# rqhuang88/DV-Matcher

Measured on AMD Instinct MI355X. Metric: point-cloud pairs/sec (N=2048, d=128), higher is better.
Workload: dtype f32; 1 GPU; BASELINE configs[1]: synthetic random pairs N=M=2048 d=128, correspondence+deform forward, both directions; deformer_weights=reference ckpt/dvmatcher_scape_r (fixture), fps_start=0, parallelism=pairs sharded over 1 GPU(s), no collective

## Files before the change

dv-matcher_amd/csrc/dvm_api.cpp:

```cpp
#include <stdarg.h>

#include "dvm_common.h"

namespace dvm {
static thread_local char g_err[512] = "";
void set_error(const char *fmt, ...) {
    va_list ap;
    va_start(ap, fmt);
    vsnprintf(g_err, sizeof(g_err), fmt, ap);
    va_end(ap);
}
}

DVM_EXPORT int dvm_abi_version(void) { return DVM_ABI_VERSION; }
DVM_EXPORT const char *dvm_last_error(void) { return dvm::g_err; }
DVM_EXPORT int dvm_device_count(void) {
    int n = 0;
    if (hipGetDeviceCount(&n) != hipSuccess) return 0;
    return n;
}

#include <atomic>
#include <stdlib.h>
namespace dvm {
// ... 13 lines not shown
static std::atomic<int> g_deterministic{options().deterministic};
bool deterministic() { return g_deterministic.load(std::memory_order_relaxed) != 0; }
}
DVM_EXPORT int dvm_set_deterministic(int on) { return dvm::g_deterministic.exchange(on ? 1 : 0); }
DVM_EXPORT int dvm_get_deterministic(void) { return dvm::g_deterministic.load(std::memory_order_relaxed); }

#include <map>
#include <mutex>
#include <utility>
namespace dvm {
static std::mutex g_attr_mu;
static std::map<std::pair<int, const void *>, int> g_attr_bytes;
void ensure_dyn_lds(const void *kernel, int bytes) {
    int dev = 0;
    if (hipGetDevice(&dev) != hipSuccess) return;
    std::lock_guard<std::mutex> lock(g_attr_mu);
    auto it = g_attr_bytes.find({dev, kernel});
    if (it != g_attr_bytes.end() && it->second >= bytes) return;
    if (hipFuncSetAttribute(kernel, hipFuncAttributeMaxDynamicSharedMemorySize, bytes) == hipSuccess) g_attr_bytes[{dev, kernel}] = bytes;
}
int device_cu_count() {
    static std::mutex mu;
    static std::map<int, int> cus;
    int dev = 0;
    if (hipGetDevice(&dev) != hipSuccess) return 256;
    std::lock_guard<std::mutex> lock(mu);
    auto it = cus.find(dev);
    if (it != cus.end()) return it->second;
    int n = 0;
    if (hipDeviceGetAttribute(&n, hipDeviceAttributeMultiprocessorCount, dev) != hipSuccess || n < 1) n = 256;
    cus[dev] = n;
    return n;
}
}

namespace dvm {
static std::mutex g_pair_mu;
static std::map<std::pair<int, hipStream_t>, PairCtx *> g_pair_ctx;
PairCtx *pair_ctx_find(hipStream_t caller) {
    int dev = 0;
    if (hipGetDevice(&dev) != hipSuccess) return nullptr;
    std::lock_guard<std::mutex> lock(g_pair_mu);
    auto it = g_pair_ctx.find({dev, caller});
    return it == g_pair_ctx.end() ? nullptr : it->second;
}
static void pair_ctx_free(PairCtx *c) {
    if (c->side) (void)hipStreamDestroy(c->side);
    if (c->side2) (void)hipStreamDestroy(c->side2);
    for (hipEvent_t e : {c->ev_fork, c->ev_join, c->ev_join2, c->ev_aux})
        if (e) (void)hipEventDestroy(e);
    delete c;
}
}

DVM_EXPORT int dvm_pair_init(void *stream) {
    int dev = 0;
    if (hipGetDevice(&dev) != hipSuccess) {
        dvm::set_error("dvm_pair_init: no current device");
        return DVM_ELAUNCH;
    }
    std::lock_guard<std::mutex> lock(dvm::g_pair_mu);
    const auto key = std::make_pair(dev, (hipStream_t)stream);
    if (dvm::g_pair_ctx.count(key)) return DVM_OK;
    dvm::PairCtx *c = new dvm::PairCtx();
    c->device = dev;
    if (hipStreamCreateWithFlags(&c->side, hipStreamNonBlocking) != hipSuccess ||
        hipStreamCreateWithFlags(&c->side2, hipStreamNonBlocking) != hipSuccess ||
// ... 150 lines not shown
```

dv-matcher_amd/csrc/dvm_common.h:

```cpp
#pragma once
#include <hip/hip_runtime.h>
#include <stdint.h>
#include <stdio.h>
#include <string.h>

#include "../../include/dvm.h"

#define DVM_EXPORT extern "C" __attribute__((visibility("default")))

namespace dvm {

void set_error(const char *fmt, ...);
void prof_begin(hipStream_t s, int id = 0);
void prof_end(hipStream_t s, int id = 0);
bool deterministic();
void prof_note(int id, const char *name);
void ensure_dyn_lds(const void *kernel, int bytes);
int device_cu_count();
struct Options {
    int deterministic;
    int k1_route;
    float k1_p_coarse, k1_p_lean;
    int linear_cfg;
    int pair_overlap;
    int debug;
};
constexpr int DVM_DEBUG_K1_ROUTES = 1, DVM_DEBUG_K1_FLAGGED = 2, DVM_DEBUG_CHAMFER_STATS = 4, DVM_DEBUG_K1_STAMPS = 8, DVM_DEBUG_MLP_STAMPS = 16;
const Options &options();
struct PairCtx {
    int device = 0;
    hipStream_t side = nullptr, side2 = nullptr;
    hipEvent_t ev_fork = nullptr, ev_join = nullptr, ev_join2 = nullptr, ev_aux = nullptr;
};
PairCtx *pair_ctx_find(hipStream_t caller);

#define DVM_REQUIRE(cond, ...)            \
    do {                                  \
        if (!(cond)) {                    \
            dvm::set_error(__VA_ARGS__);  \
            return DVM_EINVAL;            \
        }                                 \
    } while (0)

#define DVM_CHECK_LAUNCH(name)                                                          \
    do {                                                                                \
        hipError_t e_ = hipGetLastError();                                              \
        if (e_ != hipSuccess) {                                                         \
            dvm::set_error("%s: launch failed: %s", name, hipGetErrorString(e_));       \
            return DVM_ELAUNCH;                                                         \
        }                                                                               \
    } while (0)
// ... 392 lines not shown
```

dv-matcher_amd/csrc/dvm_deformer.hip:

```cpp
#include "dvm_mfma_tile.h"
#include "dvm_mlp_f16.h"

namespace dvm {


constexpr int DF_C = 128;

__global__ __launch_bounds__(256) void pool_kernel(const float *__restrict__ feat, const int32_t *__restrict__ idx,
                                                   const int32_t *__restrict__ rowmap, int P, int nrows, int k,
                                                   const float *__restrict__ cw, const float *__restrict__ cb,
                                                   float *__restrict__ out, int out_stride, int out_off,
                                                   const int32_t *__restrict__ order) {
    const int b = blockIdx.y;
    const long g = (long)blockIdx.x * blockDim.x + threadIdx.x;
    if (g >= (long)nrows * (DF_C / 4)) return;
    int r = (int)(g / (DF_C / 4));
    const int c4 = (int)(g % (DF_C / 4));
    if (order) r = order[(size_t)b * nrows + r];
    const int v = rowmap ? rowmap[(size_t)b * nrows + r] : r;
    const float *fb = feat + (size_t)b * P * DF_C;
    const int32_t *ix = idx + ((size_t)b * P + v) * k;
    f32x4 acc = {0.f, 0.f, 0.f, 0.f};
    if (k == 10) {
        int nb[10];
// ... 84 lines not shown
    } else {
#pragma unroll
        for (int t = 0; t < TOPK; ++t) {
            if (t < topk) {
                f32x4 f = *(const f32x4 *)(g2b + (size_t)pc[t] * DF_C + 4 * c4);
                acc.x = fmaf(pv[t], f.x, acc.x);
                acc.y = fmaf(pv[t], f.y, acc.y);
                acc.z = fmaf(pv[t], f.z, acc.z);
                acc.w = fmaf(pv[t], f.w, acc.w);
            }
        }
    }
    float *zr = z + ((size_t)b * Nn + n) * DF_ZS;
    zr[134 + 4 * c4] = acc.x, zr[135 + 4 * c4] = acc.y, zr[136 + 4 * c4] = acc.z, zr[137 + 4 * c4] = acc.w;
    if (c4 == 0) {
        for (int c = 0; c < 3; ++c) {
            zr[c] = verts1[row * 3 + c];
            zr[131 + c] = verts12[row * 3 + c];
        }
        zr[262] = 0.f, zr[263] = 0.f;
    }
}

struct AssembleSide {
    const float *vsrc, *vcorr, *gsrc, *gtgt, *pi_val;
    const int32_t *pi_idx, *fps;
    int N, M, Nn;
    float *z;
};
struct AssembleArgs {
    AssembleSide d[2];
    int topk;
    const int *gate;
};
template <int TOPK, bool PLANES = false>
__global__ __launch_bounds__(256) void assemble_pooled_kernel(const AssembleArgs args) {
    const int *__restrict__ gate = args.gate;
    if (gate && *gate == 0) return;
    const AssembleSide &A = args.d[blockIdx.z];
    const float *__restrict__ vsrc = A.vsrc, *__restrict__ vcorr = A.vcorr, *__restrict__ gsrc = A.gsrc, *__restrict__ gtgt = A.gtgt;
    const float *__restrict__ pi_val = A.pi_val;
    const int32_t *__restrict__ pi_idx = A.pi_idx, *__restrict__ fps = A.fps;
    const int N = A.N, M = A.M, Nn = A.Nn, topk = args.topk;
    float *__restrict__ z = A.z;
    const int b = blockIdx.y;
    const long g = (long)blockIdx.x * blockDim.x + threadIdx.x;
    if (g >= (long)Nn * (DF_C / 4)) return;
    const int n = (int)(g / (DF_C / 4)), c4 = (int)(g % (DF_C / 4));
    const int v = fps[(size_t)b * Nn + n];
    const size_t row = (size_t)b * N + v;
    const int lane = threadIdx.x & 63, base = lane & 32, l32 = lane & 31;
    const bool live = l32 < topk;
    const size_t o = row * topk + (live ? l32 : 0);
    const float pvt = pi_val[o];
    const int pct = pi_idx[o];
    const float my_pv = live ? pvt : 0.f;
    const int my_pc = live ? pct : 0x7fffffff;
    int rank = 0;
#pragma unroll
    for (int u = 0; u < TOPK; ++u) {
        const int pcu = __shfl(my_pc, base + u, 64);
        rank += (pcu < my_pc || (pcu == my_pc && u < l32)) ? 1 : 0;
    }
    const int dst = l32 < TOPK ? base + rank : lane;
    const int spc = __builtin_amdgcn_ds_permute(dst << 2, my_pc);
    const float spv = __int_as_float(__builtin_amdgcn_ds_permute(dst << 2, __float_as_int(my_pv)));
    float pv[TOPK];
    int pc[TOPK];
#pragma unroll
    for (int t = 0; t < TOPK; ++t) {
        pc[t] = __shfl(spc, base + t, 64);
        pv[t] = __shfl(spv, base + t, 64);
    }
    const float *gt = gtgt + (size_t)b * M * DF_C;
    f32x4 acc = {0.f, 0.f, 0.f, 0.f};
    if (topk == TOPK) {
        f32x4 f[TOPK];
#pragma unroll
        for (int t = 0; t < TOPK; ++t) f[t] = *(const f32x4 *)(gt + (size_t)pc[t] * DF_C + 4 * c4);
// ... 21 lines not shown
        typedef unsigned u32x2 __attribute__((ext_vector_type(2)));
        typedef unsigned u32x4 __attribute__((ext_vector_type(4)));
        char *zr = (char *)z + ((size_t)b * Nn + n) * MH_SZ;
        unsigned h0, m0, h1, m1;
        split2x2(gs.x * MH_SA, gs.y * MH_SA, h0, m0);
        split2x2(gs.z * MH_SA, gs.w * MH_SA, h1, m1);
        *(u32x2 *)(zr + 8 * c4) = u32x2{h0, h1};
        *(u32x2 *)(zr + 2 * MH_K0 + 8 * c4) = u32x2{m0, m1};
        split2x2(acc.x * MH_SA, acc.y * MH_SA, h0, m0);
        split2x2(acc.z * MH_SA, acc.w * MH_SA, h1, m1);
        *(u32x2 *)(zr + 256 + 8 * c4) = u32x2{h0, h1};
        *(u32x2 *)(zr + 2 * MH_K0 + 256 + 8 * c4) = u32x2{m0, m1};
        if (c4 == 0) {
            unsigned h2, m2;
            split2x2(vsrc[row * 3] * MH_SA, vsrc[row * 3 + 1] * MH_SA, h0, m0);
            split2x2(vsrc[row * 3 + 2] * MH_SA, vcorr[row * 3] * MH_SA, h1, m1);
            split2x2(vcorr[row * 3 + 1] * MH_SA, vcorr[row * 3 + 2] * MH_SA, h2, m2);
            *(u32x4 *)(zr + 512) = u32x4{h0, h1, h2, 0u};
            *(u32x4 *)(zr + 528) = u32x4{0u, 0u, 0u, 0u};
            *(u32x4 *)(zr + 2 * MH_K0 + 512) = u32x4{m0, m1, m2, 0u};
            *(u32x4 *)(zr + 2 * MH_K0 + 528) = u32x4{0u, 0u, 0u, 0u};
        }
        return;
    }
    float *zr = z + ((size_t)b * Nn + n) * DF_ZS;
    zr[3 + 4 * c4] = gs.x, zr[4 + 4 * c4] = gs.y, zr[5 + 4 * c4] = gs.z, zr[6 + 4 * c4] = gs.w;
    zr[134 + 4 * c4] = acc.x, zr[135 + 4 * c4] = acc.y, zr[136 + 4 * c4] = acc.z, zr[137 + 4 * c4] = acc.w;
    if (c4 == 0) {
        for (int c = 0; c < 3; ++c) {
            zr[c] = vsrc[row * 3 + c];
            zr[131 + c] = vcorr[row * 3 + c];
        }
        zr[262] = 0.f, zr[263] = 0.f;
    }
}

__device__ __forceinline__ float elu1(float x) { return x > 0.f ? x : __builtin_amdgcn_exp2f(x * 1.4426950408889634f) - 1.f; }

__global__ void mlp_layer_scalar_kernel(const float *__restrict__ in, int in_stride, const float *__restrict__ W,
                                        const float *__restrict__ bias, int rows, int I, int O, int act,
                                        float *__restrict__ out, int out_stride) {
    long g = (long)blockIdx.x * blockDim.x + threadIdx.x;
    if (g >= (long)rows * O) return;
    int r = (int)(g / O), o = (int)(g % O);
    const float *x = in + (size_t)r * in_stride, *w = W + (size_t)o * I;
    float acc = 0.f;
    for (int c = 0; c < I; ++c) acc = fmaf(x[c], w[c], acc);
    acc = acc + bias[o];
    out[(size_t)r * out_stride + o] = act ? elu1(acc) : acc;
}

__global__ void pack_weights_kernel(const float *__restrict__ W, int O, int I, int otiles, int steps, float *__restrict__ Wp) {
    long g = (long)blockIdx.x * blockDim.x + threadIdx.x;
    long total = (long)otiles * steps * 64;
    if (g >= total) return;
    int lane = (int)(g % 64);
    int step = (int)((g / 64) % steps);
    int ot = (int)(g / (64L * steps));
    int o = ot * 32 + (lane & 31), c = 2 * step + (lane >> 5);
    Wp[g] = (o < O && c < I) ? W[(size_t)o * I + c] : 0.f;
}

constexpr int ML_NODES = 32;
constexpr int ML_WAVES = 8;
constexpr int ML_THREADS = 64 * ML_WAVES;
constexpr int ML_SA = 268;
// ... 149 lines not shown
        layer(w.h0, 512, W1, b1, 512, 256, 1, w.h1, 256);
        layer(w.h1, 256, W2, b2, 256, 128, 1, w.h2, 128);
        layer(w.h2, 128, W3, b3, 128, 9, 0, out, 9);
    } else {
        launch_mlp_rows(w.z, rows, W0, b0, W1, b1, W2, b2, W3, b3, w.Wp0, out, s, variant, w.zp);
    }
    return DVM_OK;
}

__global__ void pad_rows_kernel(const float *__restrict__ in, int rows, int I, int stride, float *__restrict__ out) {
    long g = (long)blockIdx.x * blockDim.x + threadIdx.x;
    if (g >= (long)rows * stride) return;
    int r = (int)(g / stride), c = (int)(g % stride);
    out[g] = c < I ? in[(size_t)r * I + c] : 0.f;
}

void launch_pool_all(const float *feat, const int32_t *idx, int B, int P, int k, const float *cw, const float *cb, float *out,
                     hipStream_t s, const int32_t *order) {
    prof_begin(s, DVM_PROF_POOL);
    hipLaunchKernelGGL(pool_kernel, dim3((unsigned)(((long)P * 32 + 255) / 256), B), dim3(256), 0, s, feat, idx,
                       (const int32_t *)nullptr, P, P, k, cw, cb, out, DF_C, 0, order);
    prof_end(s, DVM_PROF_POOL);
}
void launch_assemble_pooled_pair(const float *verts1, const float *verts2, const float *verts12, const float *verts21, const float *g1,
                                 const float *g2, const float *val12, const int32_t *idx12, const float *val21, const int32_t *idx21,
                                 const int32_t *nodes1, const int32_t *nodes2, int B, int N, int M, void *z12, void *z21, bool planes,
                                 const int *gate, hipStream_t s) {
    AssembleArgs a;
    a.d[0] = AssembleSide{verts1, verts12, g1, g2, val12, idx12, nodes1, N, M, N / 2, (float *)z12};
    a.d[1] = AssembleSide{verts2, verts21, g2, g1, val21, idx21, nodes2, M, N, M / 2, (float *)z21};
    a.topk = 10, a.gate = gate;
    const int nn = N / 2 > M / 2 ? N / 2 : M / 2;
    const dim3 grid((unsigned)(((long)nn * 32 + 255) / 256), B, 2);
    if (!gate) prof_begin(s, DVM_PROF_ASSEMBLE);
    if (planes) hipLaunchKernelGGL((assemble_pooled_kernel<10, true>), grid, dim3(256), 0, s, a);
    else hipLaunchKernelGGL(assemble_pooled_kernel<10>, grid, dim3(256), 0, s, a);
    if (!gate) prof_end(s, DVM_PROF_ASSEMBLE);
}
const int *launch_mlp_planes(const void *zp, int rows, const float *W0, const float *b0, const float *W1, const float *b1, const float *W2,
                             const float *b2, const float *W3, const float *b3, float *wp, float *out, hipStream_t s) {
    return launch_mlp_planes_f16(zp, rows, W0, b0, W1, b1, W2, b2, W3, b3, wp, out, s);
}
void launch_mlp_fallback(const float *z, int rows, const float *W0, const float *b0, const float *W1, const float *b1, const float *W2,
                         const float *b2, const float *W3, const float *b3, float *wp, float *out, hipStream_t s, const int *flag) {
    launch_mlp_rows_bf16(z, rows, W0, b0, W1, b1, W2, b2, W3, b3, (char *)wp + mlp_f16_pack_bytes(), out, s, flag);
}
size_t mlp_pack_floats() {
    size_t f32 = (size_t)16 * 132 * 64 + (size_t)8 * 256 * 64 + (size_t)4 * 128 * 64 + (size_t)64 * 64;
    size_t h16 = (mlp_f16_pack_bytes() + mlp_bf16_pack_bytes() + 3) / 4;
    return f32 > h16 ? f32 : h16;
}
void launch_mlp_rows(const float *z, int rows, const float *W0, const float *b0, const float *W1, const float *b1, const float *W2,
                     const float *b2, const float *W3, const float *b3, float *wp, float *out, hipStream_t s, int variant, void *zp) {
    if (variant == 0 && zp) {
        launch_split_rows(z, rows, DF_ZS, zp, s);
        const int *flag = launch_mlp_planes_f16(zp, rows, W0, b0, W1, b1, W2, b2, W3, b3, wp, out, s);
        launch_mlp_rows_bf16(z, rows, W0, b0, W1, b1, W2, b2, W3, b3, (char *)wp + mlp_f16_pack_bytes(), out, s, flag);
        return;
    }
    if (variant == 0) variant = 3;
    if (variant == 3) {
        launch_mlp_rows_bf16(z, rows, W0, b0, W1, b1, W2, b2, W3, b3, wp, out, s, nullptr);
        return;
    }
    float *Wp0 = wp, *Wp1 = Wp0 + (size_t)16 * 132 * 64, *Wp2 = Wp1 + (size_t)8 * 256 * 64, *Wp3 = Wp2 + (size_t)4 * 128 * 64;
    auto pack = [&](const float *W, int O, int I, int otiles, int steps, float *Wp) {
        long th = (long)otiles * steps * 64;
        hipLaunchKernelGGL(pack_weights_kernel, dim3((unsigned)((th + 255) / 256)), dim3(256), 0, s, W, O, I, otiles, steps, Wp);
    };
// ... 56 lines not shown
```

dv-matcher_amd/csrc/dvm_mlp_bf16.hip:

```cpp
#include "dvm_mfma_tile.h"

namespace dvm {

typedef __bf16 bf16x8 __attribute__((ext_vector_type(8)));

constexpr int MB_NODES = 32, MB_WAVES = 8, MB_THREADS = 64 * MB_WAVES;
constexpr int MB_ZS = 264;
constexpr int MB_K0 = 272, MB_K1 = 512, MB_K2 = 256, MB_K3 = 128;
constexpr int MB_SA = 3 * MB_K0 * 2 + 16;
constexpr int MB_SB = 3 * MB_K1 * 2 + 16;
constexpr size_t MB_LDS_BYTES = (size_t)MB_NODES * (MB_SA + MB_SB);

__device__ __forceinline__ void split3(float x, __bf16 &h, __bf16 &m, __bf16 &l) {
    h = (__bf16)x;
    float r = x - (float)h;
    m = (__bf16)r;
    float r2 = r - (float)m;
    l = (__bf16)r2;
}

struct PackLayersBf16 {
    const float *W[4];
    int O[4], I[4], otiles[4], steps[4];
    __bf16 *Wp[4];
// ... 41 lines not shown
        acc = __builtin_amdgcn_mfma_f32_32x32x16_bf16(ah, bm, acc, 0, 0, 0);
        acc = __builtin_amdgcn_mfma_f32_32x32x16_bf16(ah, bh, acc, 0, 0, 0);
        bh = ch, bm = cm, bl = cl;
        ch = nh, cm = nm, cl = nl;
    }
    return acc;
}

__device__ __forceinline__ float elu_fast(float x) {
    return x > 0.f ? x : __builtin_amdgcn_exp2f(x * 1.4426950408889634f) - 1.f;
}

__device__ __forceinline__ void mlp_store_bf16(const f32x16 &acc, const float *__restrict__ bias, int o, int O, char *dst,
                                               int stride, int plane_bytes, int hh) {
    if (o >= O) return;
    const float bv = bias[o];
#pragma unroll
    for (int r = 0; r < 16; ++r) {
        const int node = lane_key(r, hh);
        __bf16 h, m, l;
        split3(elu_fast(acc[r] + bv), h, m, l);
        char *p = dst + node * stride + 2 * o;
        *(__bf16 *)(p) = h;
        *(__bf16 *)(p + plane_bytes) = m;
        *(__bf16 *)(p + 2 * plane_bytes) = l;
    }
}

__global__ __launch_bounds__(MB_THREADS) void mlp_bf16x3_kernel(const float *__restrict__ z, int rows,
                                                                const __bf16 *__restrict__ Wp0, const float *__restrict__ b0,
                                                                const __bf16 *__restrict__ Wp1, const float *__restrict__ b1,
                                                                const __bf16 *__restrict__ Wp2, const float *__restrict__ b2,
                                                                const __bf16 *__restrict__ Wp3, const float *__restrict__ b3,
                                                                float *__restrict__ out, const int *__restrict__ gate) {
    if (gate && *gate == 0) return;
    extern __shared__ __attribute__((aligned(16))) char smem[];
    char *bufA = smem;
    char *bufB = smem + MB_NODES * MB_SA;
    const int tid = threadIdx.x, lane = tid & 63, wave = tid >> 6;
    const int r32 = lane & 31, hh = lane >> 5;
    const int row0 = blockIdx.x * MB_NODES;

    for (int e = tid; e < MB_NODES * (MB_K0 / 4); e += MB_THREADS) {
        const int r = e / (MB_K0 / 4), c = e % (MB_K0 / 4);
        f32x4 v = {0.f, 0.f, 0.f, 0.f};
        if (row0 + r < rows && 4 * c < MB_ZS) v = *(const f32x4 *)(z + (size_t)(row0 + r) * MB_ZS + 4 * c);
        char *p = bufA + r * MB_SA + 8 * c;
#pragma unroll
        for (int q = 0; q < 4; ++q) {
            __bf16 h, m, l;
            split3(v[q], h, m, l);
            *(__bf16 *)(p + 2 * q) = h;
            *(__bf16 *)(p + 2 * MB_K0 + 2 * q) = m;
            *(__bf16 *)(p + 4 * MB_K0 + 2 * q) = l;
        }
    }
    __syncthreads();
    for (int q = 0; q < 2; ++q) {
        const int ot = wave * 2 + q;
        f32x16 acc = mlp_tile_bf16(bufA + r32 * MB_SA + 16 * hh, 2 * MB_K0, Wp0 + (size_t)ot * (MB_K0 / 16) * 1536 + lane * 8,
                                   MB_K0 / 16);
        mlp_store_bf16(acc, b0, ot * 32 + r32, 512, bufB, MB_SB, 2 * MB_K1, hh);
    }
    __syncthreads();
    {
        const int ot = wave;
        f32x16 acc = mlp_tile_bf16(bufB + r32 * MB_SB + 16 * hh, 2 * MB_K1, Wp1 + (size_t)ot * (MB_K1 / 16) * 1536 + lane * 8,
                                   MB_K1 / 16);
        mlp_store_bf16(acc, b1, ot * 32 + r32, 256, bufA, MB_SA, 2 * MB_K2, hh);
    }
    __syncthreads();
    if (wave < 4) {
        const int ot = wave;
        f32x16 acc = mlp_tile_bf16(bufA + r32 * MB_SA + 16 * hh, 2 * MB_K2, Wp2 + (size_t)ot * (MB_K2 / 16) * 1536 + lane * 8,
                                   MB_K2 / 16);
        mlp_store_bf16(acc, b2, ot * 32 + r32, 128, bufB, MB_SB, 2 * MB_K3, hh);
    }
    __syncthreads();
    if (wave == 0) {
        f32x16 acc = mlp_tile_bf16(bufB + r32 * MB_SB + 16 * hh, 2 * MB_K3, Wp3 + lane * 8, MB_K3 / 16);
        const int o = r32;
        const float bv = o < 9 ? b3[o] : 0.f;
#pragma unroll
        for (int r = 0; r < 16; ++r) {
            const int node = lane_key(r, hh);
            if (o < 9 && row0 + node < rows) out[(size_t)(row0 + node) * 9 + o] = acc[r] + bv;
        }
    }
}

size_t mlp_bf16_pack_bytes() {
    return align_up(((size_t)16 * (MB_K0 / 16) + (size_t)8 * (MB_K1 / 16) + (size_t)4 * (MB_K2 / 16) + (size_t)1 * (MB_K3 / 16)) * 1536 *
                    sizeof(__bf16));
}

void launch_mlp_rows_bf16(const float *z, int rows, const float *W0, const float *b0, const float *W1, const float *b1,
                          const float *W2, const float *b2, const float *W3, const float *b3, void *scratch, float *out,
                          hipStream_t s, const int *gate) {
    __bf16 *Wp0 = (__bf16 *)scratch;
    __bf16 *Wp1 = Wp0 + (size_t)16 * (MB_K0 / 16) * 1536;
    __bf16 *Wp2 = Wp1 + (size_t)8 * (MB_K1 / 16) * 1536;
    __bf16 *Wp3 = Wp2 + (size_t)4 * (MB_K2 / 16) * 1536;
    {
        PackLayersBf16 a;
        long maxth = 0;
        auto layer = [&](int q, const float *W, int O, int I, int otiles, int steps, __bf16 *Wp) {
            a.W[q] = W, a.O[q] = O, a.I[q] = I, a.otiles[q] = otiles, a.steps[q] = steps, a.Wp[q] = Wp;
            const long th = (long)otiles * steps * 512;
            maxth = th > maxth ? th : maxth;
        };
        layer(0, W0, 512, 262, 16, MB_K0 / 16, Wp0);
        layer(1, W1, 256, 512, 8, MB_K1 / 16, Wp1);
        layer(2, W2, 128, 256, 4, MB_K2 / 16, Wp2);
        layer(3, W3, 9, 128, 1, MB_K3 / 16, Wp3);
        hipLaunchKernelGGL(pack_layers_bf16_kernel, dim3((unsigned)((maxth + 255) / 256), 4), dim3(256), 0, s, a, gate);
    }
    ensure_dyn_lds((const void *)mlp_bf16x3_kernel, (int)MB_LDS_BYTES);
    hipLaunchKernelGGL(mlp_bf16x3_kernel, dim3((rows + MB_NODES - 1) / MB_NODES), dim3(MB_THREADS), MB_LDS_BYTES, s, z, rows, Wp0,
                       b0, Wp1, b1, Wp2, b2, Wp3, b3, out, gate);
}

}
```

dv-matcher_amd/csrc/dvm_softcorr_coarse.hip:

```cpp
#include <stdlib.h>

#include "dvm_softcorr_f16.h"

namespace dvm {
namespace k1 {
namespace {

constexpr int HC_ROWB = 256;
constexpr int HC_KL = 12;
constexpr unsigned HC_REMOVED = 0xffc00000u;
constexpr unsigned HC_KBASE = 129u << 23;
constexpr float HC_FLOOR = 4.5f;
constexpr unsigned HC_EMASK = 0xffffe00fu;
constexpr int HC_MAX_M = 256 * 32;

constexpr int HC_QB = 2;
constexpr int HC_NREC = 32;
constexpr int HC_WAVES = 4;
template <int KT, int W> constexpr int hc_lds_bytes() { return 2 * KT * HC_ROWB + 2 * KT * 32 + 1024 + W * HC_QB * HC_NREC * 64 * 2; }

struct HCGroup {
    const char *qp, *kp;
    const char *knf;
    const float *nq;
// ... 126 lines not shown
#pragma unroll
        for (int s = 0; s < 8; ++s) qh[qb][s] = -*(const f16x8 *)(qptr + 32 * s);
        const float nas = norm_scaled(G.nq[(size_t)b * N + qrc], se);
        const float nasb = (nas + nas * 0x1p-8f) + HC_FLOOR;
        rowc[qb] = nasb - nas;
        qn[qb] = f16x8{0, 0, 0, 0, 0, 0, 0, 0};
        if (h == 0) {
            _Float16 p1, p2, p3;
            norm_pieces(nasb, p1, p2, p3);
            qn[qb][0] = (_Float16)0x1p+15f, qn[qb][1] = (_Float16)0x1p+4f, qn[qb][2] = (_Float16)0x1p-7f;
            qn[qb][3] = p1, qn[qb][4] = p2, qn[qb][5] = p3;
        }
    }

    List32<HC_KL> kb[QB];
#pragma unroll
    for (int qb = 0; qb < QB; ++qb) kb[qb].init();

    const int ntiles = (M + KT - 1) / KT, nsub = SUBS * ntiles;
    const int rgrp = (nsub + NREC - 1) / NREC;
    unsigned short *const rec = rec0 + (size_t)wave * QB * NREC * 64 + lane;
    unsigned urec[QB];
#pragma unroll
    for (int qb = 0; qb < QB; ++qb) urec[qb] = 0xffffffffu;

    const __amdgpu_buffer_rsrc_t krs = __builtin_amdgcn_make_buffer_rsrc((void *)kbase, 0, M * HB_ROWB, 0x00020000);
    const __amdgpu_buffer_rsrc_t nrs = __builtin_amdgcn_make_buffer_rsrc((void *)nfbase, 0, G.Mpad * 32, 0x00020000);
    auto stage_tile = [&](int t, int buf, bool clamp) __attribute__((always_inline)) {
        int lane;
        asm volatile("v_mbcnt_lo_u32_b32 %0, -1, 0\n\tv_mbcnt_hi_u32_b32 %0, -1, %0" : "=v"(lane));
        const int j0 = t * KT;
        char *kt = ktile0 + (size_t)buf * KT * HC_ROWB;
        constexpr int PIECES = KT * HC_ROWB / 1024 / W, NP = KT * 32 / 1024;
#pragma unroll
        for (int e = 0; e < PIECES; ++e) {
            const int piece = wave * PIECES + e;
            const int r = 4 * piece + (lane >> 4), rc = clamp ? min(r, M - 1 - j0) : r;
            const unsigned off = rc * HB_ROWB + (((lane & 15) ^ (r & 15)) << 4);
            __builtin_amdgcn_raw_ptr_buffer_load_lds(krs, (__attribute__((address_space(3))) void *)(kt + piece * 1024), 16, off, j0 * HB_ROWB, 0, 0);
        }
        __builtin_amdgcn_raw_ptr_buffer_load_lds(nrs, (__attribute__((address_space(3))) void *)(wave < NP ? knf0 + buf * KT * 32 + wave * 1024 : dump0), 16,
                                                 (wave < NP ? wave : 0) * 1024 + lane * 16, j0 * 32, 0, 0);
    };
    auto dma_barrier = [&]() __attribute__((always_inline)) {
        asm volatile("s_waitcnt vmcnt(0)" ::: "memory");
        __syncthreads();
    };

    unsigned fadr[8];
    {
        const unsigned rowb = (unsigned)(size_t)(const __attribute__((address_space(3))) char *)ktile0 + r32 * HC_ROWB;
        const int tq = h ^ (r32 & 15);
#pragma unroll
        for (int s = 0; s < 8; ++s) {
            fadr[s] = rowb + (((2 * s) ^ tq) << 4);
            asm volatile("" : "+v"(fadr[s]));
        }
    }
    unsigned nadr = (unsigned)(size_t)(const __attribute__((address_space(3))) char *)knf0 + r32 * 32 + 16 * h;
    asm volatile("" : "+v"(nadr));
    auto lds16 = [](unsigned adr, int off) __attribute__((always_inline)) {
        return *(const f16x8 *)(const __attribute__((address_space(3))) char *)(size_t)(adr + off);
    };
    struct Acc {
        f32x16 a[QB];
    };
    auto chain = [&](int buf, int sub) __attribute__((always_inline)) -> Acc {
        const int toff = buf * (KT * HC_ROWB) + sub * (32 * HC_ROWB);
        Acc A;
#pragma unroll
        for (int qb = 0; qb < QB; ++qb) A.a[qb] = f32x16{0.f, 0.f, 0.f, 0.f, 0.f, 0.f, 0.f, 0.f, 0.f, 0.f, 0.f, 0.f, 0.f, 0.f, 0.f, 0.f};
#pragma unroll
        for (int s = 0; s < 8; ++s) {
            const f16x8 fr = lds16(fadr[s], toff);
#pragma unroll
// ... 335 lines not shown
```

dv-matcher_amd/csrc/dvm_softcorr_f16.hip:

```cpp
#include "dvm_softcorr_f16.h"

namespace dvm {
namespace {

using namespace k1;

template <bool LEAN, bool CHECK_ROUTE = true>
__device__ __forceinline__ void sweep_f16_block(const HBArgs &args, int block, int nblocks, char *smem_b) {
    char *const ktile0 = smem_b;
    float *const knorm0 = (float *)(smem_b + (size_t)2 * HB_KT * HB_ROWB);
    float *const stage = knorm0 + 2 * HB_KT + (threadIdx.x >> 6) * HB_STAGE + (threadIdx.x & 63);

    int lid = xcd_remap(block, nblocks);
    const int grp = lid >= args.blocks0 ? 1 : 0;
    lid -= grp ? args.blocks0 : 0;
    const HBGroup &G = args.g[grp];
    const int N = G.N, M = G.M;
    const int b = lid / G.tiles, qt = lid % G.tiles;
    if (CHECK_ROUTE && args.route && args.route[grp * args.nb + b] != (LEAN ? K1_ROUTE_LEAN : K1_ROUTE_FULL)) return;
    const float neg_alpha = args.neg_alpha;
    const int tid = threadIdx.x, lane = tid & 63, wave = tid >> 6;
    const int r32 = lane & 31, h = lane >> 5;

    const char *kbase = G.kp + (size_t)b * M * HB_ROWB;
// ... 149 lines not shown
        __syncthreads();
    }

    {
        const float co = __shfl_xor(cref, 32, 64), lo = __shfl_xor(l, 32, 64);
        const float cm = fmaxf(cref, co);
        const float a = (cref == -INFINITY) ? 0.f : l * exp2f((cref - cm) * LOG2E);
        const float bb = (co == -INFINITY) ? 0.f : lo * exp2f((co - cm) * LOG2E);
        l = a + bb;
        cref = cm;
        double other[HB_KC];
#pragma unroll
        for (int t = 0; t < HB_KC; ++t)
            other[t] = __hiloint2double(__shfl_xor(__double2hiint(kb.e[t]), 32, 64), __shfl_xor(__double2loint(kb.e[t]), 32, 64));
#pragma unroll
        for (int t = 0; t < HB_KC; ++t) add_term(PackedBest<HB_KC>::key_of(kb.insert(other[t])));
    }
    if (h == 0 && qrow < N) {
        const size_t row = (size_t)b * N + qrow;
#pragma unroll
        for (int t = 0; t < HB_KC; ++t) {
            G.cidx[row * HB_KC + t] = PackedBest<HB_KC>::col_of(kb.e[t]);
            G.cd2[row * HB_KC + t] = kb.key(t);
        }
        G.lsum[row * 2] = l;
        G.lsum[row * 2 + 1] = cref;
    }
}
template <bool LEAN>
__global__ __launch_bounds__(HB_THREADS, 2) void softcorr_sweep_f16_kernel(const HBArgs args) {
    extern __shared__ __attribute__((aligned(16))) char smem_b[];
    sweep_f16_block<LEAN>(args, blockIdx.x, gridDim.x, smem_b);
}
__global__ __launch_bounds__(HB_THREADS, 2) void softcorr_sweep_f16_routed_kernel(const HBArgs args) {
    extern __shared__ __attribute__((aligned(16))) char smem_b[];
    int lid = xcd_remap(blockIdx.x, gridDim.x);
    const int grp = lid >= args.blocks0 ? 1 : 0;
    lid -= grp ? args.blocks0 : 0;
    const int route = args.route[grp * args.nb + lid / args.g[grp].tiles];
    if (route == K1_ROUTE_LEAN) sweep_f16_block<true, false>(args, blockIdx.x, gridDim.x, smem_b);
    else if (route == K1_ROUTE_FULL) sweep_f16_block<false, false>(args, blockIdx.x, gridDim.x, smem_b);
}
__global__ __launch_bounds__(HB_THREADS, 2) void softcorr_sweep_f16_gated_kernel(const HBArgs args, int nblocks) {
    extern __shared__ __attribute__((aligned(16))) char smem_b[];
    const bool on0 = args.route[0] == K1_ROUTE_LEAN, on1 = nblocks > args.blocks0 && args.route[args.nb] == K1_ROUTE_LEAN;
    if (!on0 && !on1) return;
    for (int vb = blockIdx.x; vb < nblocks; vb += gridDim.x) {
        sweep_f16_block<true>(args, vb, nblocks, smem_b);
        __syncthreads();
    }
}

}

void k1::launch_sweep_f16(const HBArgs &a, int blocks, int form, hipStream_t s) {
    auto go = [&](auto kernel, int grid, auto... more) {
        ensure_dyn_lds((const void *)kernel, (int)HB_LDS_BYTES);
        hipLaunchKernelGGL(kernel, dim3(grid), dim3(HB_THREADS), HB_LDS_BYTES, s, a, more...);
    };
    if (form == K1_SWEEP_ROUTED) go(softcorr_sweep_f16_routed_kernel, blocks);
    else if (form == K1_SWEEP_GATED) go(softcorr_sweep_f16_gated_kernel, blocks < 2048 ? blocks : 2048, blocks);
    else if (form == K1_ROUTE_LEAN) go(softcorr_sweep_f16_kernel<true>, blocks);
    else go(softcorr_sweep_f16_kernel<false>, blocks);
}

}
```

include/dvm.h:

```cpp
#ifndef DVM_H
#define DVM_H

#include <stddef.h>
#include <stdint.h>

#ifdef __cplusplus
extern "C" {
#endif

#define DVM_ABI_VERSION 1

#define DVM_OK 0
#define DVM_EINVAL (-1)
#define DVM_ELAUNCH (-2)
#define DVM_ENOSPACE (-3)

typedef int (*dvm_allreduce_fn)(void *user, void *buf, size_t count, int dtype, int op, void *stream);
typedef struct dvm_collective {
    dvm_allreduce_fn allreduce;
    void *user;
} dvm_collective;


int dvm_abi_version(void);
// ... 8 lines not shown
#define DVM_PROF_KNN_XYZ 5
#define DVM_PROF_FPS 6
#define DVM_PROF_ASSEMBLE 7
#define DVM_PROF_COUNT 8
int dvm_profile_enable(int max_launches);
int dvm_profile_select(unsigned kernel_mask);
int dvm_profile_read(double *total_ms, int *launches);
int dvm_profile_read_kernel(int kernel, double *total_ms, int *launches);
const char *dvm_profile_kernel_name(int kernel);
int dvm_profile_disable(void);

int dvm_rownorm2_f32(const float *x, int rows, int K, float *out, void *stream);

int dvm_linear_f32(const float *x, const float *w, int B, int N, int K, int Co, int channel_major, const float *bias,
                   const float *res, const float *bn_alpha, const float *bn_beta, float slope, float *y, void *stream);

int dvm_linear_prefix_f32(const float *xg, int Cg, const float *x, const float *w, int B, int N, int K, int Co,
                          const float *bias, const float *res, const float *bn_alpha, const float *bn_beta, float slope,
                          float *y, void *stream);

int dvm_linear_scaled_residual_f32(const float *x, const float *w, int B, int N, int K, int Co, int channel_major, const float *bias,
                                   float scale, const float *res, float *y, void *stream);

int dvm_linear_last_launch(int *info);

int dvm_linear_wgrad_f32(const float *gy, const float *x, long R, int Co, int K, float *dW, void *stream);
size_t dvm_linear_wgrad_workspace_bytes(long R, int Co, int K);
int dvm_linear_wgrad_ws_f32(const float *gy, const float *x, long R, int Co, int K, float *dW, void *ws, size_t ws_bytes, void *stream);

int dvm_set_deterministic(int on);
int dvm_get_deterministic(void);

int dvm_k1_last_routes(int *counts);

size_t dvm_softcorr_workspace_bytes(int B, int N, int M, int d);
int dvm_softcorr_fwd_f32(const float *f1, const float *f2, int B, int N, int M, int d, float neg_alpha, int topk,
                         float *pi_val, int32_t *pi_idx, float *row_smax, float *row_sum, int variant, void *ws,
                         size_t ws_bytes, void *stream);

size_t dvm_sinkhorn_workspace_bytes(int B, int N, int M, int d);
int dvm_sinkhorn_fwd_f32(const float *f1, const float *f2, int B, int N, int M, int d, float neg_alpha, int n_iter,
                         int topk, float *pi_val, int32_t *pi_idx, float *row_lmax, float *row_sum, float *u, float *v,
                         int variant, void *ws, size_t ws_bytes, void *stream);

size_t dvm_sinkhorn_hist_workspace_bytes(int B, int N, int M, int d);
int dvm_sinkhorn_fwd_hist_f32(const float *f1, const float *f2, int B, int N, int M, int d, float neg_alpha, int n_iter,
                              int topk, float *pi_val, int32_t *pi_idx, float *row_lmax, float *row_sum, float *u_hist,
                              float *v_hist, int variant, void *ws, size_t ws_bytes, void *stream);
size_t dvm_sinkhorn_bwd_workspace_bytes(int B, int N, int M, int d, int n_iter);
int dvm_sinkhorn_bwd_f32(const float *f1, const float *f2, int B, int N, int M, int d, float neg_alpha, int n_iter, int topk,
                         const float *pi_val, const int32_t *pi_idx, const float *u_hist, const float *v_hist,
                         const float *g_val, float *d_f1, float *d_f2, int variant, void *ws, size_t ws_bytes,
                         void *stream);

size_t dvm_sinkhorn_ub_workspace_bytes(int B, int N, int M, int d);
int dvm_sinkhorn_ub_fwd_f32(const float *f1, const float *f2, int B, int N, int M, int d, float neg_alpha, int n_iter, int topk,
                            float tau_row, float tau_col, const float *log_a, const float *log_b, float *pi_val,
                            int32_t *pi_idx, float *row_lmax, float *row_sum, float *row_lmass, float *u, float *v, int variant,
                            void *ws, size_t ws_bytes, void *stream);
size_t dvm_sinkhorn_ub_hist_workspace_bytes(int B, int N, int M, int d);
int dvm_sinkhorn_ub_fwd_hist_f32(const float *f1, const float *f2, int B, int N, int M, int d, float neg_alpha, int n_iter,
                                 int topk, float tau_row, float tau_col, const float *log_a, const float *log_b, float *pi_val,
                                 int32_t *pi_idx, float *row_lmax, float *row_sum, float *row_lmass, float *rn_hist,
                                 float *cn_hist, int variant, void *ws, size_t ws_bytes, void *stream);
size_t dvm_sinkhorn_ub_bwd_workspace_bytes(int B, int N, int M, int d, int n_iter);
int dvm_sinkhorn_ub_bwd_f32(const float *f1, const float *f2, int B, int N, int M, int d, float neg_alpha, int n_iter, int topk,
// ... 308 lines not shown
```

Baseline: 58290 pairs/s.

## Cap gated kernel grids to CU-proportional persistent loops with early exit

Converts the gated assemble, bf16 MLP and routed f16 sweep kernels into grid-stride persistent loops whose grid size is a per-CU multiple, so fully-gated or mostly-skipped launches no longer spawn thousands of idle workgroups. The routed sweep first scans the route table block-wide and exits early when every tile is coarse. The coarse softcorr DMA loader also gets a simpler, precomputed swizzled offset for the unclamped path. The trade-off is that fewer resident workgroups may underfill the GPU when the gated work is actually live, and the added loop barriers and route scan add overhead.

Result: no change. 57720 pairs/s (median of 2 runs) (-1.0%).

```diff
diff --git a/dv-matcher_amd/csrc/dvm_api.cpp b/dv-matcher_amd/csrc/dvm_api.cpp
--- a/dv-matcher_amd/csrc/dvm_api.cpp
+++ b/dv-matcher_amd/csrc/dvm_api.cpp
@@ -69,7 +69,15 @@
     cus[dev] = n;
     return n;
 }
-}
+static std::atomic<int> g_gated_grid{0};
+int gated_grid(int items, int per_cu) {
+    const int o = g_gated_grid.load(std::memory_order_relaxed);
+    if (o > 0) return o;
+    const long want = o < 0 ? items : (long)per_cu * device_cu_count();
+    return (int)(want < items ? want : items > 0 ? items : 1);
+}
+}
+DVM_EXPORT int dvm_debug_set_gated_grid(int workgroups) { return dvm::g_gated_grid.exchange(workgroups); }
 
 namespace dvm {
 static std::mutex g_pair_mu;
diff --git a/dv-matcher_amd/csrc/dvm_common.h b/dv-matcher_amd/csrc/dvm_common.h
--- a/dv-matcher_amd/csrc/dvm_common.h
+++ b/dv-matcher_amd/csrc/dvm_common.h
@@ -17,6 +17,7 @@
 void prof_note(int id, const char *name);
 void ensure_dyn_lds(const void *kernel, int bytes);
 int device_cu_count();
+int gated_grid(int items, int per_cu);
 struct Options {
     int deterministic;
     int k1_route;
diff --git a/dv-matcher_amd/csrc/dvm_deformer.hip b/dv-matcher_amd/csrc/dvm_deformer.hip
--- a/dv-matcher_amd/csrc/dvm_deformer.hip
+++ b/dv-matcher_amd/csrc/dvm_deformer.hip
@@ -140,19 +140,17 @@
     AssembleSide d[2];
     int topk;
     const int *gate;
+    int nx, B;
 };
-template <int TOPK, bool PLANES = false>
-__global__ __launch_bounds__(256) void assemble_pooled_kernel(const AssembleArgs args) {
-    const int *__restrict__ gate = args.gate;
-    if (gate && *gate == 0) return;
-    const AssembleSide &A = args.d[blockIdx.z];
+template <int TOPK, bool PLANES>
+__device__ __forceinline__ void assemble_pooled_item(const AssembleArgs &args, unsigned bx, int b, unsigned side) {
+    const AssembleSide &A = args.d[side];
     const float *__restrict__ vsrc = A.vsrc, *__restrict__ vcorr = A.vcorr, *__restrict__ gsrc = A.gsrc, *__restrict__ gtgt = A.gtgt;
     const float *__restrict__ pi_val = A.pi_val;
     const int32_t *__restrict__ pi_idx = A.pi_idx, *__restrict__ fps = A.fps;
     const int N = A.N, M = A.M, Nn = A.Nn, topk = args.topk;
     float *__restrict__ z = A.z;
-    const int b = blockIdx.y;
-    const long g = (long)blockIdx.x * blockDim.x + threadIdx.x;
+    const long g = (long)bx * blockDim.x + threadIdx.x;
     if (g >= (long)Nn * (DF_C / 4)) return;
     const int n = (int)(g / (DF_C / 4)), c4 = (int)(g % (DF_C / 4));
     const int v = fps[(size_t)b * Nn + n];
@@ -240,6 +238,20 @@
             zr[131 + c] = vcorr[row * 3 + c];
         }
         zr[262] = 0.f, zr[263] = 0.f;
+    }
+}
+template <int TOPK, bool PLANES = false>
+__global__ __launch_bounds__(256) void assemble_pooled_kernel(const AssembleArgs args) {
+    const int *__restrict__ gate = args.gate;
+    if (gate && *gate == 0) return;
+    if constexpr (PLANES) {
+        assemble_pooled_item<TOPK, true>(args, blockIdx.x, blockIdx.y, blockIdx.z);
+    } else {
+        const int per_side = args.nx * args.B;
+        for (int it = blockIdx.x; it < 2 * per_side; it += gridDim.x) {
+            const int side = it >= per_side ? 1 : 0, r = it - side * per_side;
+            assemble_pooled_item<TOPK, false>(args, r % args.nx, r / args.nx, side);
+        }
     }
 }
 
@@ -455,9 +467,11 @@
     a.topk = 10, a.gate = gate;
     const int nn = N / 2 > M / 2 ? N / 2 : M / 2;
     const dim3 grid((unsigned)(((long)nn * 32 + 255) / 256), B, 2);
+    a.nx = (int)grid.x, a.B = B;
+    const int items = 2 * a.nx * B;
     if (!gate) prof_begin(s, DVM_PROF_ASSEMBLE);
     if (planes) hipLaunchKernelGGL((assemble_pooled_kernel<10, true>), grid, dim3(256), 0, s, a);
-    else hipLaunchKernelGGL(assemble_pooled_kernel<10>, grid, dim3(256), 0, s, a);
+    else hipLaunchKernelGGL(assemble_pooled_kernel<10>, dim3(gate ? gated_grid(items, 8) : items), dim3(256), 0, s, a);
     if (!gate) prof_end(s, DVM_PROF_ASSEMBLE);
 }
 const int *launch_mlp_planes(const void *zp, int rows, const float *W0, const float *b0, const float *W1, const float *b1, const float *W2,
diff --git a/dv-matcher_amd/csrc/dvm_mlp_bf16.hip b/dv-matcher_amd/csrc/dvm_mlp_bf16.hip
--- a/dv-matcher_amd/csrc/dvm_mlp_bf16.hip
+++ b/dv-matcher_amd/csrc/dvm_mlp_bf16.hip
@@ -97,60 +97,64 @@
                                                                 const __bf16 *__restrict__ Wp1, const float *__restrict__ b1,
                                                                 const __bf16 *__restrict__ Wp2, const float *__restrict__ b2,
                                                                 const __bf16 *__restrict__ Wp3, const float *__restrict__ b3,
-                                                                float *__restrict__ out, const int *__restrict__ gate) {
+                                                                float *__restrict__ out, const int *__restrict__ gate, int nblocks) {
     if (gate && *gate == 0) return;
     extern __shared__ __attribute__((aligned(16))) char smem[];
     char *bufA = smem;
     char *bufB = smem + MB_NODES * MB_SA;
     const int tid = threadIdx.x, lane = tid & 63, wave = tid >> 6;
     const int r32 = lane & 31, hh = lane >> 5;
-    const int row0 = blockIdx.x * MB_NODES;
+    for (int vb = blockIdx.x; vb < nblocks; vb += gridDim.x) {
+        const int row0 = vb * MB_NODES;
+        asm volatile("" : "+s"(Wp0), "+s"(Wp1), "+s"(Wp2), "+s"(Wp3));
 
-    for (int e = tid; e < MB_NODES * (MB_K0 / 4); e += MB_THREADS) {
-        const int r = e / (MB_K0 / 4), c = e % (MB_K0 / 4);
-        f32x4 v = {0.f, 0.f, 0.f, 0.f};
-        if (row0 + r < rows && 4 * c < MB_ZS) v = *(const f32x4 *)(z + (size_t)(row0 + r) * MB_ZS + 4 * c);
-        char *p = bufA + r * MB_SA + 8 * c;
+        for (int e = tid; e < MB_NODES * (MB_K0 / 4); e += MB_THREADS) {
+            const int r = e / (MB_K0 / 4), c = e % (MB_K0 / 4);
+            f32x4 v = {0.f, 0.f, 0.f, 0.f};
+            if (row0 + r < rows && 4 * c < MB_ZS) v = *(const f32x4 *)(z + (size_t)(row0 + r) * MB_ZS + 4 * c);
+            char *p = bufA + r * MB_SA + 8 * c;
 #pragma unroll
-        for (int q = 0; q < 4; ++q) {
-            __bf16 h, m, l;
-            split3(v[q], h, m, l);
-            *(__bf16 *)(p + 2 * q) = h;
-            *(__bf16 *)(p + 2 * MB_K0 + 2 * q) = m;
-            *(__bf16 *)(p + 4 * MB_K0 + 2 * q) = l;
+            for (int q = 0; q < 4; ++q) {
+                __bf16 h, m, l;
+                split3(v[q], h, m, l);
+                *(__bf16 *)(p + 2 * q) = h;
+                *(__bf16 *)(p + 2 * MB_K0 + 2 * q) = m;
+                *(__bf16 *)(p + 4 * MB_K0 + 2 * q) = l;
+            }
         }
-    }
-    __syncthreads();
-    for (int q = 0; q < 2; ++q) {
-        const int ot = wave * 2 + q;
-        f32x16 acc = mlp_tile_bf16(bufA + r32 * MB_SA + 16 * hh, 2 * MB_K0, Wp0 + (size_t)ot * (MB_K0 / 16) * 1536 + lane * 8,
-                                   MB_K0 / 16);
-        mlp_store_bf16(acc, b0, ot * 32 + r32, 512, bufB, MB_SB, 2 * MB_K1, hh);
-    }
-    __syncthreads();
-    {
-        const int ot = wave;
-        f32x16 acc = mlp_tile_bf16(bufB + r32 * MB_SB + 16 * hh, 2 * MB_K1, Wp1 + (size_t)ot * (MB_K1 / 16) * 1536 + lane * 8,
-                                   MB_K1 / 16);
-        mlp_store_bf16(acc, b1, ot * 32 + r32, 256, bufA, MB_SA, 2 * MB_K2, hh);
-    }
-    __syncthreads();
-    if (wave < 4) {
-        const int ot = wave;
-        f32x16 acc = mlp_tile_bf16(bufA + r32 * MB_SA + 16 * hh, 2 * MB_K2, Wp2 + (size_t)ot * (MB_K2 / 16) * 1536 + lane * 8,
-                                   MB_K2 / 16);
-        mlp_store_bf16(acc, b2, ot * 32 + r32, 128, bufB, MB_SB, 2 * MB_K3, hh);
-    }
-    __syncthreads();
-    if (wave == 0) {
-        f32x16 acc = mlp_tile_bf16(bufB + r32 * MB_SB + 16 * hh, 2 * MB_K3, Wp3 + lane * 8, MB_K3 / 16);
-        const int o = r32;
-        const float bv = o < 9 ? b3[o] : 0.f;
+        __syncthreads();
+        for (int q = 0; q < 2; ++q) {
+            const int ot = wave * 2 + q;
+            f32x16 acc = mlp_tile_bf16(bufA + r32 * MB_SA + 16 * hh, 2 * MB_K0, Wp0 + (size_t)ot * (MB_K0 / 16) * 1536 + lane * 8,
+                                       MB_K0 / 16);
+            mlp_store_bf16(acc, b0, ot * 32 + r32, 512, bufB, MB_SB, 2 * MB_K1, hh);
+        }
+        __syncthreads();
+        {
+            const int ot = wave;
+            f32x16 acc = mlp_tile_bf16(bufB + r32 * MB_SB + 16 * hh, 2 * MB_K1, Wp1 + (size_t)ot * (MB_K1 / 16) * 1536 + lane * 8,
+                                       MB_K1 / 16);
+            mlp_store_bf16(acc, b1, ot * 32 + r32, 256, bufA, MB_SA, 2 * MB_K2, hh);
+        }
+        __syncthreads();
+        if (wave < 4) {
+            const int ot = wave;
+            f32x16 acc = mlp_tile_bf16(bufA + r32 * MB_SA + 16 * hh, 2 * MB_K2, Wp2 + (size_t)ot * (MB_K2 / 16) * 1536 + lane * 8,
+                                       MB_K2 / 16);
+            mlp_store_bf16(acc, b2, ot * 32 + r32, 128, bufB, MB_SB, 2 * MB_K3, hh);
+        }
+        __syncthreads();
+        if (wave == 0) {
+            f32x16 acc = mlp_tile_bf16(bufB + r32 * MB_SB + 16 * hh, 2 * MB_K3, Wp3 + lane * 8, MB_K3 / 16);
+            const int o = r32;
+            const float bv = o < 9 ? b3[o] : 0.f;
 #pragma unroll
-        for (int r = 0; r < 16; ++r) {
-            const int node = lane_key(r, hh);
-            if (o < 9 && row0 + node < rows) out[(size_t)(row0 + node) * 9 + o] = acc[r] + bv;
+            for (int r = 0; r < 16; ++r) {
+                const int node = lane_key(r, hh);
+                if (o < 9 && row0 + node < rows) out[(size_t)(row0 + node) * 9 + o] = acc[r] + bv;
+            }
         }
+        __syncthreads();
     }
 }
 
@@ -181,8 +185,9 @@
         hipLaunchKernelGGL(pack_layers_bf16_kernel, dim3((unsigned)((maxth + 255) / 256), 4), dim3(256), 0, s, a, gate);
     }
     ensure_dyn_lds((const void *)mlp_bf16x3_kernel, (int)MB_LDS_BYTES);
-    hipLaunchKernelGGL(mlp_bf16x3_kernel, dim3((rows + MB_NODES - 1) / MB_NODES), dim3(MB_THREADS), MB_LDS_BYTES, s, z, rows, Wp0,
-                       b0, Wp1, b1, Wp2, b2, Wp3, b3, out, gate);
+    const int nblocks = (rows + MB_NODES - 1) / MB_NODES;
+    hipLaunchKernelGGL(mlp_bf16x3_kernel, dim3(gate ? gated_grid(nblocks, 2) : nblocks), dim3(MB_THREADS), MB_LDS_BYTES, s, z, rows, Wp0,
+                       b0, Wp1, b1, Wp2, b2, Wp3, b3, out, gate, nblocks);
 }
 
 }
diff --git a/dv-matcher_amd/csrc/dvm_softcorr_coarse.hip b/dv-matcher_amd/csrc/dvm_softcorr_coarse.hip
--- a/dv-matcher_amd/csrc/dvm_softcorr_coarse.hip
+++ b/dv-matcher_amd/csrc/dvm_softcorr_coarse.hip
@@ -182,15 +182,21 @@
         const int j0 = t * KT;
         char *kt = ktile0 + (size_t)buf * KT * HC_ROWB;
         constexpr int PIECES = KT * HC_ROWB / 1024 / W, NP = KT * 32 / 1024;
+        const unsigned base = (lane >> 4) * HB_ROWB + (((lane & 15) ^ (lane >> 4)) << 4);
 #pragma unroll
         for (int e = 0; e < PIECES; ++e) {
             const int piece = wave * PIECES + e;
-            const int r = 4 * piece + (lane >> 4), rc = clamp ? min(r, M - 1 - j0) : r;
-            const unsigned off = rc * HB_ROWB + (((lane & 15) ^ (r & 15)) << 4);
-            __builtin_amdgcn_raw_ptr_buffer_load_lds(krs, (__attribute__((address_space(3))) void *)(kt + piece * 1024), 16, off, j0 * HB_ROWB, 0, 0);
+            if (clamp) {
+                const int r = 4 * piece + (lane >> 4), rc = min(r, M - 1 - j0);
+                const unsigned off = rc * HB_ROWB + (((lane & 15) ^ (r & 15)) << 4);
+                __builtin_amdgcn_raw_ptr_buffer_load_lds(krs, (__attribute__((address_space(3))) void *)(kt + piece * 1024), 16, off, j0 * HB_ROWB, 0, 0);
+            } else {
+                __builtin_amdgcn_raw_ptr_buffer_load_lds(krs, (__attribute__((address_space(3))) void *)(kt + piece * 1024), 16, base ^ ((piece & 3) << 6),
+                                                         (j0 + 4 * piece) * HB_ROWB, 0, 0);
+            }
         }
         __builtin_amdgcn_raw_ptr_buffer_load_lds(nrs, (__attribute__((address_space(3))) void *)(wave < NP ? knf0 + buf * KT * 32 + wave * 1024 : dump0), 16,
-                                                 (wave < NP ? wave : 0) * 1024 + lane * 16, j0 * 32, 0, 0);
+                                                 lane * 16, j0 * 32 + (wave < NP ? wave : 0) * 1024, 0, 0);
     };
     auto dma_barrier = [&]() __attribute__((always_inline)) {
         asm volatile("s_waitcnt vmcnt(0)" ::: "memory");
diff --git a/dv-matcher_amd/csrc/dvm_softcorr_f16.hip b/dv-matcher_amd/csrc/dvm_softcorr_f16.hip
--- a/dv-matcher_amd/csrc/dvm_softcorr_f16.hip
+++ b/dv-matcher_amd/csrc/dvm_softcorr_f16.hip
@@ -205,14 +205,20 @@
     extern __shared__ __attribute__((aligned(16))) char smem_b[];
     sweep_f16_block<LEAN>(args, blockIdx.x, gridDim.x, smem_b);
 }
-__global__ __launch_bounds__(HB_THREADS, 2) void softcorr_sweep_f16_routed_kernel(const HBArgs args) {
+__global__ __launch_bounds__(HB_THREADS, 2) void softcorr_sweep_f16_routed_kernel(const HBArgs args, int nblocks) {
     extern __shared__ __attribute__((aligned(16))) char smem_b[];
-    int lid = xcd_remap(blockIdx.x, gridDim.x);
-    const int grp = lid >= args.blocks0 ? 1 : 0;
-    lid -= grp ? args.blocks0 : 0;
-    const int route = args.route[grp * args.nb + lid / args.g[grp].tiles];
-    if (route == K1_ROUTE_LEAN) sweep_f16_block<true, false>(args, blockIdx.x, gridDim.x, smem_b);
-    else if (route == K1_ROUTE_FULL) sweep_f16_block<false, false>(args, blockIdx.x, gridDim.x, smem_b);
+    int mine = 0;
+    for (int i = threadIdx.x; i < (nblocks > args.blocks0 ? 2 : 1) * args.nb; i += HB_THREADS) mine |= args.route[i] != K1_ROUTE_COARSE;
+    if (!__syncthreads_or(mine)) return;
+    for (int vb = blockIdx.x; vb < nblocks; vb += gridDim.x) {
+        int lid = xcd_remap(vb, nblocks);
+        const int grp = lid >= args.blocks0 ? 1 : 0;
+        lid -= grp ? args.blocks0 : 0;
+        const int route = args.route[grp * args.nb + lid / args.g[grp].tiles];
+        if (route == K1_ROUTE_LEAN) sweep_f16_block<true, false>(args, vb, nblocks, smem_b);
+        else if (route == K1_ROUTE_FULL) sweep_f16_block<false, false>(args, vb, nblocks, smem_b);
+        __syncthreads();
+    }
 }
 __global__ __launch_bounds__(HB_THREADS, 2) void softcorr_sweep_f16_gated_kernel(const HBArgs args, int nblocks) {
     extern __shared__ __attribute__((aligned(16))) char smem_b[];
@@ -231,7 +237,7 @@
         ensure_dyn_lds((const void *)kernel, (int)HB_LDS_BYTES);
         hipLaunchKernelGGL(kernel, dim3(grid), dim3(HB_THREADS), HB_LDS_BYTES, s, a, more...);
     };
-    if (form == K1_SWEEP_ROUTED) go(softcorr_sweep_f16_routed_kernel, blocks);
+    if (form == K1_SWEEP_ROUTED) go(softcorr_sweep_f16_routed_kernel, gated_grid(blocks, 4), blocks);
     else if (form == K1_SWEEP_GATED) go(softcorr_sweep_f16_gated_kernel, blocks < 2048 ? blocks : 2048, blocks);
     else if (form == K1_ROUTE_LEAN) go(softcorr_sweep_f16_kernel<true>, blocks);
     else go(softcorr_sweep_f16_kernel<false>, blocks);
diff --git a/include/dvm.h b/include/dvm.h
--- a/include/dvm.h
+++ b/include/dvm.h
@@ -64,6 +64,8 @@
 int dvm_get_deterministic(void);
 
 int dvm_k1_last_routes(int *counts);
+
+int dvm_debug_set_gated_grid(int workgroups);
 
 size_t dvm_softcorr_workspace_bytes(int B, int N, int M, int d);
 int dvm_softcorr_fwd_f32(const float *f1, const float *f2, int B, int N, int M, int d, float neg_alpha, int topk,
```
